# bababyVN/medical-image-segmentation-and-classification

Measured on AMD Instinct MI355X. Metric: images/sec (train step) Attention U-Net 256x256 bs=32/GPU, higher is better.
Workload: dtype bf16; 1 GPU; AttentionUNet 256x256 train step (fwd+BCE+bwd+clip+AdamW), bs=32/GPU, NHWC bf16 activations, fp32 master weights; global_batch=32, parallelism=dp1, hip_graph=False, wgrad_side_stream=True, plan_replay=C (mi355_plan_run)

## Files before the change

### medical-image-segmentation-and-classification_amd/csrc/bn.hip

```cpp
#include "rowred.hpp"

template <typename T> struct BnStatsOp {
  static constexpr int NQ = 2;
  static constexpr bool WRITES = false;
  typedef double Acc;
  static constexpr int EPC = 16 / (int)sizeof(T);
  const T* x;
  int ld;
  __device__ void load_cols(int) {}
  __device__ void apply(size_t row, int c0, Acc (&acc)[NQ][EPC]) const {
    const Vec16<T> v = ld16<T>(x + row * ld + c0);
#pragma unroll
    for (int e = 0; e < EPC; ++e) {
      const double f = (double)to_f32<T>(v.v[e]);
      acc[0][e] += f;
      acc[1][e] += f * f;
    }
  }
};


template <int CH, int BL, int NQ>
__device__ __forceinline__ void fold_partials(const float* __restrict__ partial, int nblocks, int rowlen, const int (&off)[NQ], int C,
                                              double* red , double (&out)[NQ]) {
  static_assert(CH * BL == 1024 && CH <= 64 && (CH & (CH - 1)) == 0, "1024-thread workgroup, power-of-two channel count");
  const int cl = threadIdx.x % CH, bl = threadIdx.x / CH;
  const int c = blockIdx.x * CH + cl;
  const int wave = threadIdx.x >> 6, lane = threadIdx.x & 63;
  double s[NQ];
#pragma unroll
  for (int q = 0; q < NQ; ++q) {
    double s0 = 0, s1 = 0, s2 = 0, s3 = 0;
    if (c < C) {
      const float* p = partial + off[q] + c;
      int b = bl;
      for (; b + 3 * BL < nblocks; b += 4 * BL) {
        s0 += (double)p[(size_t)b * rowlen];
        s1 += (double)p[(size_t)(b + BL) * rowlen];
        s2 += (double)p[(size_t)(b + 2 * BL) * rowlen];
        s3 += (double)p[(size_t)(b + 3 * BL) * rowlen];
      }
      for (; b < nblocks; b += BL) s0 += (double)p[(size_t)b * rowlen];
    }
    s[q] = (s0 + s1) + (s2 + s3);
  }
#pragma unroll
  for (int q = 0; q < NQ; ++q) {
#pragma unroll
    for (int m = CH; m < 64; m <<= 1) s[q] += __shfl_xor(s[q], m, 64);
    if (lane < CH) red[(q * 16 + wave) * CH + lane] = s[q];
  }
  __syncthreads();
#pragma unroll
  for (int q = 0; q < NQ; ++q) {
    double t = 0;
    if (threadIdx.x < CH) {
#pragma unroll
      for (int w = 0; w < 16; ++w) t += red[(q * 16 + w) * CH + threadIdx.x];
    }
    out[q] = t;
  }
}

extern "C" int mi355_rowreduce_blocks(long long M) { return rowreduce_blocks(M); }

extern "C" int mi355_bn_stats(const void* x, float* partial, long long M, int C, int ld, int dtype, mi355_stream_t s) {
  MI355_CHECK_ARG(x && partial && M > 0, "bn_stats: bad arguments");
  return dispatch_dtype(dtype, "bn_stats", [&](auto tag) {
    using T = decltype(tag);
    BnStatsOp<T> op{(const T*)x, ld};
    return rowred_launch<T>(op, M, C, partial, (hipStream_t)s);
  });
}

template <int CH, int BL>
__global__ __launch_bounds__(1024) void bn_finalize_kernel(const float* __restrict__ partial, int nblocks, double M, int C,
                                   const float* __restrict__ gamma, const float* __restrict__ beta,
                                   float* __restrict__ rmean, float* __restrict__ rvar, int64_t* nbt, float momentum,
                                   float eps, float* __restrict__ scale, float* __restrict__ shift,
                                   float* __restrict__ mean_out, float* __restrict__ invstd_out) {
  __shared__ double red[2 * 16 * CH];
  double sums2[2];
  fold_partials<CH, BL, 2>(partial, nblocks, 2 * C, {0, C}, C, red, sums2);
  const double s = sums2[0], q = sums2[1];
  const int c = blockIdx.x * CH + threadIdx.x;
  if (threadIdx.x >= CH) return;
  if (c == 0 && nbt) *nbt += 1;
  if (c >= C) return;
  const double mean = s / M;
  double var = q / M - mean * mean;
  if (var < 0) var = 0;
  const float invstd = (float)(1.0 / sqrt(var + (double)eps));
  if (rmean) {
    const double unb = M > 1 ? var * M / (M - 1) : var;
    rmean[c] = (float)((1.0 - momentum) * rmean[c] + momentum * mean);
    rvar[c] = (float)((1.0 - momentum) * rvar[c] + momentum * unb);
  }
  const float sc = gamma[c] * invstd;
  scale[c] = sc;
  shift[c] = beta[c] - (float)mean * sc;
  mean_out[c] = (float)mean;
  invstd_out[c] = invstd;
}

extern "C" int mi355_bn_finalize(const float* partial, int nblocks, long long M, int C, const float* gamma,
                                 const float* beta, float* running_mean, float* running_var, int64_t* nbt,
                                 float momentum, float eps, float* scale, float* shift, float* mean, float* invstd,
                                 mi355_stream_t s) {
  MI355_CHECK_ARG(partial && gamma && beta && scale && shift && mean && invstd, "bn_finalize: null pointer");
  if (nblocks > 128)
    hipLaunchKernelGGL((bn_finalize_kernel<4, 256>), dim3(ceil_div(C, 4)), dim3(1024), 0, (hipStream_t)s, partial, nblocks, (double)M, C,
                       gamma, beta, running_mean, running_var, nbt, momentum, eps, scale, shift, mean, invstd);
  else
    hipLaunchKernelGGL((bn_finalize_kernel<32, 32>), dim3(ceil_div(C, 32)), dim3(1024), 0, (hipStream_t)s, partial, nblocks, (double)M, C,
                       gamma, beta, running_mean, running_var, nbt, momentum, eps, scale, shift, mean, invstd);
  MI355_LAUNCH_CHECK();
  return MI355_OK;
}

__global__ __launch_bounds__(256) void fold_rows_kernel(const float* __restrict__ in, int rows, int rowlen, float* __restrict__ out,
                                                        int nsplit) {
  __shared__ double red[4][64];
  const int cl = threadIdx.x & 63, rl = threadIdx.x >> 6;
  const int c = blockIdx.x * 64 + cl;
  const int per = (rows + nsplit - 1) / nsplit;
  const int r0 = blockIdx.y * per, r1 = min(rows, r0 + per);
  double s0 = 0, s1 = 0, s2 = 0, s3 = 0;
  if (c < rowlen) {
    int r = r0 + rl;
    for (; r + 12 < r1; r += 16) {
      s0 += (double)in[(size_t)r * rowlen + c];
      s1 += (double)in[(size_t)(r + 4) * rowlen + c];
      s2 += (double)in[(size_t)(r + 8) * rowlen + c];
      s3 += (double)in[(size_t)(r + 12) * rowlen + c];
    }
    for (; r < r1; r += 4) s0 += (double)in[(size_t)r * rowlen + c];
  }
  red[rl][cl] = (s0 + s1) + (s2 + s3);
  __syncthreads();
  if (rl == 0 && c < rowlen) out[(size_t)blockIdx.y * rowlen + c] = (float)((red[0][cl] + red[1][cl]) + (red[2][cl] + red[3][cl]));
}

extern "C" int mi355_fold_rows(const float* partial, int rows, int rowlen, float* out, int nsplit, mi355_stream_t s) {
  MI355_CHECK_ARG(partial && out && rows > 0 && rowlen > 0 && nsplit > 0 && nsplit <= rows, "fold_rows: bad arguments");
  hipLaunchKernelGGL(fold_rows_kernel, dim3(ceil_div(rowlen, 64), nsplit), dim3(256), 0, (hipStream_t)s, partial, rows, rowlen, out,
                     nsplit);
  MI355_LAUNCH_CHECK();
  return MI355_OK;
}

__global__ void bn_eval_coeffs_kernel(const float* gamma, const float* beta, const float* rm, const float* rv, float eps,
                                      int C, float* scale, float* shift) {
  const int c = blockIdx.x * blockDim.x + threadIdx.x;
  if (c >= C) return;
  const float sc = gamma[c] / sqrtf(rv[c] + eps);
  scale[c] = sc;
  shift[c] = beta[c] - rm[c] * sc;
}

__global__ void bn_fold_bias_kernel(const float* bias, const float* scale, const float* shift, float* out, int C) {
  const int c = blockIdx.x * blockDim.x + threadIdx.x;
  if (c < C) out[c] = scale[c] * (bias ? bias[c] : 0.f) + shift[c];
}

extern "C" int mi355_bn_fold_bias(const float* bias, const float* scale, const float* shift, float* out, int C, mi355_stream_t s) {
  MI355_CHECK_ARG(scale && shift && out && C > 0, "bn_fold_bias: bad arguments");
  hipLaunchKernelGGL(bn_fold_bias_kernel, dim3(ceil_div(C, 128)), dim3(128), 0, (hipStream_t)s, bias, scale, shift, out, C);
  MI355_LAUNCH_CHECK();
  return MI355_OK;
}

extern "C" int mi355_bn_eval_coeffs(const float* gamma, const float* beta, const float* running_mean,
                                    const float* running_var, float eps, int C, float* scale, float* shift,
                                    mi355_stream_t s) {
  hipLaunchKernelGGL(bn_eval_coeffs_kernel, dim3(ceil_div(C, 128)), dim3(128), 0, (hipStream_t)s, gamma, beta, running_mean,
                     running_var, eps, C, scale, shift);
  MI355_LAUNCH_CHECK();
  return MI355_OK;
}

template <typename T, bool H2 = false, bool HR = false> struct BnActOp {
  static constexpr int EPC = 16 / (int)sizeof(T);
  const T* x; int ldx; const float* scale; const float* shift;
  const T* x2; int ldx2; const float* scale2; const float* shift2;
  const T* res; int ldr;
  T* y; int ldy;
  int act;
  float sc[EPC], sh[EPC], sc2[EPC];
  __device__ void load_cols(int c0) {
#pragma unroll
    for (int e = 0; e < EPC; ++e) {
      sc[e] = scale ? scale[c0 + e] : 1.f;
      sh[e] = scale ? shift[c0 + e] : 0.f;
      sc2[e] = H2 ? scale2[c0 + e] : 0.f;
      if constexpr (H2) sh[e] += shift2[c0 + e];
    }
  }
#ifndef BN_ACT_FETCH
#define BN_ACT_FETCH 8
#endif
  static constexpr int FETCH_ROWS = BN_ACT_FETCH;
  struct In { Vec16<T> v, v2, vr; };
  __device__ In fetch(size_t row, int c0) const {
    In in;
    in.v = ld16_nt<T>(x + row * ldx + c0);
    if constexpr (H2) in.v2 = ld16<T>(x2 + row * ldx2 + c0);
    if constexpr (HR) in.vr = ld16<T>(res + row * ldr + c0);
    return in;
  }
  __device__ void pin(In& in) const {
    pin16(in.v);
    if constexpr (H2) pin16(in.v2);
    if constexpr (HR) pin16(in.vr);
  }
  __device__ void finish(const In& in, size_t row, int c0) const {
    float f[EPC];
#pragma unroll
    for (int e = 0; e < EPC; ++e) f[e] = __builtin_fmaf(to_f32<T>(in.v.v[e]), sc[e], sh[e]);
    if constexpr (H2) {
#pragma unroll
      for (int e = 0; e < EPC; ++e) f[e] = __builtin_fmaf(to_f32<T>(in.v2.v[e]), sc2[e], f[e]);
    }
    const bool relu = act & 1, post = act & 2;
    Vec16<T> o;
#pragma unroll
    for (int e = 0; e < EPC; ++e) {
      float v = f[e];
      if (HR && !post) v += to_f32<T>(in.vr.v[e]);
      if (relu) v = fmaxf(v, 0.f);
      if (HR && post) v += to_f32<T>(in.vr.v[e]);
      o.v[e] = from_f32<T>(v);
    }
    st16<T>(y + row * ldy + c0, o);
  }
};

extern "C" int mi355_bn_act(const void* x, int ldx, const float* scale, const float* shift, const void* x2, int ldx2,
                            const float* scale2, const float* shift2, const void* res, int ldr, void* y, int ldy,
                            long long M, int C, int act, int dtype, mi355_stream_t s) {
  MI355_CHECK_ARG(x && y && M > 0, "bn_act: bad arguments");
  MI355_CHECK_ARG(!x2 || (scale2 && shift2), "bn_act: second operand needs scale2/shift2");
  return dispatch_dtype(dtype, "bn_act", [&](auto tag) {
    using T = decltype(tag);
    auto run = [&](auto op) {
      op.x = (const T*)x; op.ldx = ldx; op.scale = scale; op.shift = shift; op.x2 = (const T*)x2; op.ldx2 = ldx2;
      op.scale2 = scale2; op.shift2 = shift2; op.res = (const T*)res; op.ldr = ldr; op.y = (T*)y; op.ldy = ldy; op.act = act;
      return rowmap_launch<T>(op, M, C, (hipStream_t)s);
    };
    if (x2) return res ? run(BnActOp<T, true, true>{}) : run(BnActOp<T, true, false>{});
    return res ? run(BnActOp<T, false, true>{}) : run(BnActOp<T, false, false>{});
  });
}

#ifndef BN_ACT_POOL_WGS
#define BN_ACT_POOL_WGS 16
#endif
template <typename T, bool HR>
__global__ __launch_bounds__(256) void bn_act_pool2_kernel(const T* __restrict__ x, int ldx, const float* __restrict__ scale,
                                                           const float* __restrict__ shift, T* __restrict__ y, int ldy,
                                                           T* __restrict__ p, int ldp, int N, int H, int W, int C, int act,
                                                           const T* __restrict__ res = nullptr, int ldr = 0) {
  constexpr int EPC = 16 / (int)sizeof(T);
  const int cp = C / EPC, Ho = H >> 1, Wo = W >> 1;
  const long long total = (long long)N * Ho * Wo * cp;
  for (long long i = (long long)blockIdx.x * blockDim.x + threadIdx.x; i < total; i += (long long)gridDim.x * blockDim.x) {
    const int c0 = (int)(i % cp) * EPC;
    long long q = i / cp;
    const int wo = (int)(q % Wo); q /= Wo;
    const int ho = (int)(q % Ho);
    const int n = (int)(q / Ho);
    float sc[EPC], sh[EPC], m[EPC];
#pragma unroll
    for (int e = 0; e < EPC; ++e) { sc[e] = scale[c0 + e]; sh[e] = shift[c0 + e]; }
    const size_t r0 = ((size_t)(n * H + 2 * ho) * W + 2 * wo);
    Vec16<T> in[4];
#pragma unroll
    for (int k = 0; k < 4; ++k)
      in[k] = ld16_nt<T>(x + (r0 + (size_t)(k >> 1) * W + (k & 1)) * ldx + c0);
    Vec16<T> rs[4];
    if constexpr (HR) {
#pragma unroll
      for (int k = 0; k < 4; ++k) rs[k] = ld16<T>(res + (r0 + (size_t)(k >> 1) * W + (k & 1)) * ldr + c0);
    }
#pragma unroll
    for (int k = 0; k < 4; ++k) {
      Vec16<T> o;
#pragma unroll
      for (int e = 0; e < EPC; ++e) {
        float v = __builtin_fmaf(to_f32<T>(in[k].v[e]), sc[e], sh[e]);
        if (HR && !(act & 2)) v += to_f32<T>(rs[k].v[e]);
        if (act & 1) v = fmaxf(v, 0.f);
        if (HR && (act & 2)) v += to_f32<T>(rs[k].v[e]);
        o.v[e] = from_f32<T>(v);
        const float r = to_f32<T>(o.v[e]);
        m[e] = k == 0 ? r : fmaxf(m[e], r);
      }
      st16<T>(y + (r0 + (size_t)(k >> 1) * W + (k & 1)) * ldy + c0, o);
    }
    if (p) {
      Vec16<T> o;
#pragma unroll
      for (int e = 0; e < EPC; ++e) o.v[e] = from_f32<T>(m[e]);
      st16<T>(p + ((size_t)(n * Ho + ho) * Wo + wo) * ldp + c0, o);
    }
  }
}

extern "C" int mi355_bn_act_pool2(const void* x, int ldx, const float* scale, const float* shift, void* y, int ldy, void* p, int ldp,
                                  int N, int H, int W, int C, int act, int dtype, mi355_stream_t s) {
  MI355_CHECK_ARG(x && scale && shift && y && N > 0, "bn_act_pool2: bad arguments");
  MI355_CHECK_ARG(H % 2 == 0 && W % 2 == 0, "bn_act_pool2: %d x %d is not divisible into 2 x 2 groups", H, W);
  const int epc = dtype_is_2byte(dtype) ? 8 : 4;
  MI355_CHECK_ARG(C % epc == 0, "bn_act_pool2: C=%d must be a multiple of %d", C, epc);
  long long blocks = ((long long)N * (H / 2) * (W / 2) * (C / epc) + 255) / 256;
  if (blocks > 256 * BN_ACT_POOL_WGS) blocks = 256 * BN_ACT_POOL_WGS;
  return dispatch_dtype(dtype, "bn_act_pool2", [&](auto tag) {
    using T = decltype(tag);
    hipLaunchKernelGGL((bn_act_pool2_kernel<T, false>), dim3((int)blocks), dim3(256), 0, (hipStream_t)s, (const T*)x, ldx, scale, shift, (T*)y, ldy,
                       (T*)p, ldp, N, H, W, C, act);
    MI355_LAUNCH_CHECK();
    return (int)MI355_OK;
  });
}

extern "C" int mi355_bn_act_windows(const void* x, int ldx, const float* scale, const float* shift, const void* res, int ldr, void* y,
                                    int ldy, int N, int H, int W, int C, int act, int dtype, mi355_stream_t s) {
  MI355_CHECK_ARG(x && scale && shift && y && N > 0, "bn_act_windows: bad arguments");
  MI355_CHECK_ARG(H % 2 == 0 && W % 2 == 0, "bn_act_windows: %d x %d is not divisible into 2 x 2 groups", H, W);
  const int epc = dtype_is_2byte(dtype) ? 8 : 4;
  MI355_CHECK_ARG(C % epc == 0, "bn_act_windows: C=%d must be a multiple of %d", C, epc);
  long long blocks = ((long long)N * (H / 2) * (W / 2) * (C / epc) + 255) / 256;
  if (blocks > 256 * BN_ACT_POOL_WGS) blocks = 256 * BN_ACT_POOL_WGS;
  return dispatch_dtype(dtype, "bn_act_windows", [&](auto tag) {
    using T = decltype(tag);
    if (res)
      hipLaunchKernelGGL((bn_act_pool2_kernel<T, true>), dim3((int)blocks), dim3(256), 0, (hipStream_t)s, (const T*)x, ldx, scale, shift,
                         (T*)y, ldy, (T*)nullptr, 0, N, H, W, C, act, (const T*)res, ldr);
    else
      hipLaunchKernelGGL((bn_act_pool2_kernel<T, false>), dim3((int)blocks), dim3(256), 0, (hipStream_t)s, (const T*)x, ldx, scale, shift,
                         (T*)y, ldy, (T*)nullptr, 0, N, H, W, C, act, (const T*)nullptr, 0);
    MI355_LAUNCH_CHECK();
    return (int)MI355_OK;
  });
}

static inline long long bn_keep_limit() {
  static const long long mb = getenv("MI355_BN_KEEP_MB") ? atoll(getenv("MI355_BN_KEEP_MB")) : 0;
  return mb > 0 ? mb * 1000000ll : 0;
}
static inline int bn_reduce_keeps(long long bytes = 0) {
  static const int nt = getenv("MI355_BN_REDUCE_NT") ? atoi(getenv("MI355_BN_REDUCE_NT")) : 0;
  if (bn_keep_limit() && bytes > bn_keep_limit()) return 0;
  return nt ? 0 : 1;
}

static inline int bn_apply_keeps(long long bytes = 0) {
  static const int nt = getenv("MI355_BN_APPLY_NT") ? atoi(getenv("MI355_BN_APPLY_NT")) : 0;
  static const int lim = getenv("MI355_BN_KEEP_APPLY") ? atoi(getenv("MI355_BN_KEEP_APPLY")) : 0;
  if (lim && bn_keep_limit() && bytes > bn_keep_limit()) return 0;
  return nt ? 0 : 1;
}

static inline int bn_apply_reversed() {
  static const int rev = getenv("MI355_BN_APPLY_REV") ? atoi(getenv("MI355_BN_APPLY_REV")) : 0;
  return rev;
}

template <typename T, bool HASY = false, bool KEEP = true> struct BnBwdReduceOp {
  static constexpr int NQ = 2;
  static constexpr bool WRITES = false;
  typedef float Acc;
  static constexpr int EPC = 16 / (int)sizeof(T);
  const T* dy; int lddy; const T* y; int ldy; const T* x; int ldx;
  const float* mean; const float* invstd; const float* mscale; const float* mshift; int act;
  float mu[EPC], is[EPC], ms[EPC], mt[EPC];
  __device__ void load_cols(int c0) {
#pragma unroll
    for (int e = 0; e < EPC; ++e) {
      mu[e] = mean[c0 + e];
      is[e] = invstd[c0 + e];
      ms[e] = (act && !HASY) ? mscale[c0 + e] : 0.f;
      mt[e] = (act && !HASY) ? mshift[c0 + e] : 0.f;
    }
  }
#ifndef BN_RED_FETCH
#define BN_RED_FETCH 4
#endif
  static constexpr int FETCH_ROWS = BN_RED_FETCH;
#ifdef BN_RED_WGS
  static constexpr int MAX_WGS = BN_RED_WGS;
#endif
  struct In { Vec16<T> g, xv, yv; };
  __device__ In fetch(size_t row, int c0) const {
    In in;
    in.g = ld16_pol<KEEP, T>(dy + row * lddy + c0);
    in.xv = ld16_pol<KEEP, T>(x + row * ldx + c0);
    if constexpr (HASY) in.yv = ld16<T>(y + row * ldy + c0);
    return in;
  }
  __device__ void pin(In& in) const {
    pin16(in.g);
    pin16(in.xv);
    if constexpr (HASY) pin16(in.yv);
  }
  __device__ void finish(const In& in, size_t, int, Acc (&acc)[NQ][EPC]) const {
#pragma unroll
    for (int e = 0; e < EPC; ++e) {
      float gg = to_f32<T>(in.g.v[e]);
      const float xf = to_f32<T>(in.xv.v[e]);
      if (act) {
        const bool on = HASY ? (to_f32<T>(in.yv.v[e]) > 0.f) : (__builtin_fmaf(xf, ms[e], mt[e]) > 0.f);
        if (!on) gg = 0.f;
      }
      acc[0][e] += gg;
      acc[1][e] += gg * (xf - mu[e]) * is[e];
    }
  }
};

extern "C" int mi355_bn_bwd_reduce_rows(long long M) { return rowred_grid<BnBwdReduceOp<bf16_t>>(M); }

extern "C" int mi355_bn_bwd_reduce(const void* dy, int lddy, const void* y, int ldy, const void* x, int ldx,
                                   const float* mean, const float* invstd, const float* mscale, const float* mshift,
                                   float* partial, long long M, int C, int act, int dtype, mi355_stream_t s) {
  MI355_CHECK_ARG(dy && x && mean && invstd && partial && (!act || y || (mscale && mshift)), "bn_bwd_reduce: null pointer");
  return dispatch_dtype(dtype, "bn_bwd_reduce", [&](auto tag) {
    using T = decltype(tag);
    const bool keep = bn_reduce_keeps(2ll * M * C * (long long)sizeof(T)), hasy = act && y;
    auto run = [&](auto op) {
      op.dy = (const T*)dy; op.lddy = lddy; op.y = (const T*)y; op.ldy = ldy; op.x = (const T*)x; op.ldx = ldx;
      op.mean = mean; op.invstd = invstd; op.mscale = mscale; op.mshift = mshift; op.act = act;
      return rowred_launch<T>(op, M, C, partial, (hipStream_t)s);
    };
    if (hasy) return keep ? run(BnBwdReduceOp<T, true, true>{}) : run(BnBwdReduceOp<T, true, false>{});
    return keep ? run(BnBwdReduceOp<T, false, true>{}) : run(BnBwdReduceOp<T, false, false>{});
  });
}

template <int CH, int BL>
__global__ __launch_bounds__(1024) void bn_bwd_finalize_kernel(const float* __restrict__ partial, int nblocks, int C,
                                                               float* __restrict__ sums, float* __restrict__ dgamma,
                                                               float* __restrict__ dbeta, float accf, int nq, int q0, int q1) {
  __shared__ double red[2 * 16 * CH];
  double sums2[2];
  fold_partials<CH, BL, 2>(partial, nblocks, nq * C, {q0 * C, q1 * C}, C, red, sums2);
  const double s0 = sums2[0], s1 = sums2[1];
  const int c = blockIdx.x * CH + threadIdx.x;
  if (threadIdx.x >= CH || c >= C) return;
  sums[c] = (float)s0;
  sums[C + c] = (float)s1;
  if (dbeta) dbeta[c] = (accf != 0.f ? accf * dbeta[c] : 0.f) + (float)s0;
  if (dgamma) dgamma[c] = (accf != 0.f ? accf * dgamma[c] : 0.f) + (float)s1;
}

extern "C" int mi355_bn_bwd_finalize_at(const float* partial, int nblocks, int nq, int q0, int q1, int C, float* sums, float* dgamma,
                                        float* dbeta, float acc, mi355_stream_t s) {
  MI355_CHECK_ARG(partial && sums, "bn_bwd_finalize: null pointer");
  MI355_CHECK_ARG(nq >= 2 && q0 >= 0 && q0 < nq && q1 >= 0 && q1 < nq, "bn_bwd_finalize: quantities %d, %d of %d per partial row", q0, q1, nq);
  if (nblocks > 128)
    hipLaunchKernelGGL((bn_bwd_finalize_kernel<4, 256>), dim3(ceil_div(C, 4)), dim3(1024), 0, (hipStream_t)s, partial, nblocks, C,
                       sums, dgamma, dbeta, acc, nq, q0, q1);
  else
    hipLaunchKernelGGL((bn_bwd_finalize_kernel<32, 32>), dim3(ceil_div(C, 32)), dim3(1024), 0, (hipStream_t)s, partial, nblocks, C,
                       sums, dgamma, dbeta, acc, nq, q0, q1);
  MI355_LAUNCH_CHECK();
  return MI355_OK;
}

extern "C" int mi355_bn_bwd_finalize(const float* partial, int nblocks, int C, float* sums, float* dgamma, float* dbeta,
                                     float acc, mi355_stream_t s) {
  return mi355_bn_bwd_finalize_at(partial, nblocks, 2, 0, 1, C, sums, dgamma, dbeta, acc, s);
}

template <typename T, int NEX = 0, bool HASY = false, bool PACC = false, bool KEEP = true> struct BnBwdApplyOp {
  static constexpr int NQ = 1;
  static constexpr bool WRITES = true;
  typedef float Acc;
  static constexpr int EPC = 16 / (int)sizeof(T);
  static constexpr int NEXA = NEX > 0 ? NEX : 1;
  const T* dy; int lddy; const T* y; int ldy; const T* x; int ldx;
  const float* gamma; const float* mean; const float* invstd; const float* mscale; const float* mshift; const float* sums;
  T* dx; int lddx; T* dres; int lddres; T* dpost; int lddpost; int post_acc;
  float invM; int C; int act;
  long long last;
  const T* ex[NEXA]; int ldex, nex;
  float mu[EPC], is[EPC], k0[EPC], k1[EPC], gi[EPC], ms[EPC], mt[EPC];
  __device__ void load_cols(int c0) {
#pragma unroll
    for (int e = 0; e < EPC; ++e) {
      ms[e] = (act && !y) ? mscale[c0 + e] : 0.f;
      mt[e] = (act && !y) ? mshift[c0 + e] : 0.f;
      mu[e] = mean[c0 + e];
      is[e] = invstd[c0 + e];
      gi[e] = gamma[c0 + e] * is[e];
      k0[e] = sums[c0 + e] * invM;
      k1[e] = sums[C + c0 + e] * invM;
    }
  }
#ifndef BN_APPLY_FETCH
#define BN_APPLY_FETCH 4
#endif
  static constexpr int FETCH_ROWS = NEX > 0 ? 2 : BN_APPLY_FETCH;
  struct In { Vec16<T> g, xv, yv, pv, ev[NEXA]; };
  __device__ In fetch(size_t row, int c0) const {
    In in;
    if (last >= 0) row = (size_t)last - row;
    in.g = ld16_pol<KEEP, T>(dy + row * lddy + c0);
    in.xv = ld16_pol<KEEP, T>(x + row * ldx + c0);
    if constexpr (HASY) in.yv = ld16<T>(y + row * ldy + c0);
    if constexpr (PACC) in.pv = ld16<T>(dpost + row * lddpost + c0);
    if constexpr (NEX > 0) {
#pragma unroll
      for (int j = 0; j < NEX; ++j) in.ev[j] = ld16_nt<T>(ex[j] + row * ldex + c0);
    }
    return in;
  }
  __device__ void pin(In& in) const {
    pin16(in.g);
    pin16(in.xv);
    if constexpr (HASY) pin16(in.yv);
    if constexpr (PACC) pin16(in.pv);
    if constexpr (NEX > 0) {
#pragma unroll
      for (int j = 0; j < NEX; ++j) pin16(in.ev[j]);
    }
  }
  __device__ void finish(const In& in, size_t row, int c0, Acc (&acc)[NQ][EPC]) const {
    if (last >= 0) row = (size_t)last - row;
    if (dpost) {
      Vec16<T> pg = in.g;
      if constexpr (PACC || NEX > 0) {
#pragma unroll
        for (int e = 0; e < EPC; ++e) {
          float v = to_f32<T>(in.g.v[e]);
          if constexpr (PACC) v += to_f32<T>(in.pv.v[e]);
          if constexpr (NEX > 0) {
#pragma unroll
            for (int j = 0; j < NEX; ++j)
              if (j < nex) v += to_f32<T>(in.ev[j].v[e]);
          }
          pg.v[e] = from_f32<T>(v);
        }
      }
      st16<T>(dpost + row * lddpost + c0, pg);
    }
    Vec16<T> o, r;
#pragma unroll
    for (int e = 0; e < EPC; ++e) {
      float gg = to_f32<T>(in.g.v[e]);
      const float xf = to_f32<T>(in.xv.v[e]);
      if (act) {
        const bool on = HASY ? (to_f32<T>(in.yv.v[e]) > 0.f) : (__builtin_fmaf(xf, ms[e], mt[e]) > 0.f);
        if (!on) gg = 0.f;
      }
      const float xh = (xf - mu[e]) * is[e];
      const float d = bn_dx(gi[e], gg, k0[e], xh, k1[e]);
      o.v[e] = from_f32<T>(d);
      r.v[e] = from_f32<T>(gg);
      acc[0][e] += d;
    }
    st16<T>(dx + row * lddx + c0, o);
    if (dres) st16<T>(dres + row * lddres + c0, r);
  }
};

template <typename T, int NEX, bool HASY, bool PACC, bool KEEP>
static int bn_bwd_apply_launch(const void* dy, int lddy, const void* y, int ldy, const void* x, int ldx,
                               const float* gamma, const float* mean, const float* invstd, const float* mscale,
                               const float* mshift, const float* sums, void* dx, int lddx, void* dres, int lddres,
                               void* dpost, int lddpost, const void* const* ex, int ldex,
                               float* dbias_partial, long long M, int C, int act, mi355_stream_t s) {
  const float invM = (float)(1.0 / (double)M);
  const long long last = bn_apply_reversed() ? M - 1 : -1ll;
  BnBwdApplyOp<T, NEX, HASY, PACC, KEEP> op{(const T*)dy, lddy, (const T*)y, ldy, (const T*)x, ldx, gamma, mean, invstd,
                                            mscale, mshift, sums, (T*)dx, lddx, (T*)dres, lddres, (T*)dpost, lddpost, PACC ? 1 : 0, invM, C,
                                            act, last, {nullptr}, ldex, 0};
  if constexpr (NEX > 0) {
    for (int j = 0; j < NEX; ++j) {
      op.ex[j] = (const T*)(ex[j] ? ex[j] : ex[0]);
      if (ex[j]) op.nex = j + 1;
    }
  }
  return rowred_launch<T>(op, M, C, dbias_partial, (hipStream_t)s);
}

static int bn_bwd_apply_impl(const void* dy, int lddy, const void* y, int ldy, const void* x, int ldx,
                             const float* gamma, const float* mean, const float* invstd, const float* mscale,
                             const float* mshift, const float* sums, void* dx, int lddx, void* dres, int lddres,
                             void* dpost, int lddpost, int post_acc, const void* const* ex, int ldex,
                             float* dbias_partial, long long M, int C, int act, int dtype, mi355_stream_t s) {
  MI355_CHECK_ARG(dy && x && gamma && mean && invstd && sums && dx && (!act || y || (mscale && mshift)), "bn_bwd_apply: null pointer");
  if (ex) {
    for (int j = 1; j < 4; ++j) MI355_CHECK_ARG(!ex[j] || ex[j - 1], "bn_bwd_apply_post4: the earlier gradients must be given without gaps");
  }
  return dispatch_dtype(dtype, "bn_bwd_apply", [&](auto tag) {
    using T = decltype(tag);
    const bool hasy = act && y, pacc = dpost && post_acc;
    const bool keep = bn_apply_keeps(2ll * M * C * (long long)sizeof(T));
#define MI355_APPLY(NEX, HASY, PACC)                                                                                                       \
  (keep ? bn_bwd_apply_launch<T, NEX, HASY, PACC, true>(dy, lddy, y, ldy, x, ldx, gamma, mean, invstd, mscale, mshift, sums, dx, lddx,     \
                                                        dres, lddres, dpost, lddpost, ex, ldex, dbias_partial, M, C, act, s)               \
        : bn_bwd_apply_launch<T, NEX, HASY, PACC, false>(dy, lddy, y, ldy, x, ldx, gamma, mean, invstd, mscale, mshift, sums, dx, lddx,    \
                                                         dres, lddres, dpost, lddpost, ex, ldex, dbias_partial, M, C, act, s))
    if (ex) {
      if (hasy) return pacc ? MI355_APPLY(4, true, true) : MI355_APPLY(4, true, false);
      return pacc ? MI355_APPLY(4, false, true) : MI355_APPLY(4, false, false);
    }
    if (hasy) return pacc ? MI355_APPLY(0, true, true) : MI355_APPLY(0, true, false);
    return pacc ? MI355_APPLY(0, false, true) : MI355_APPLY(0, false, false);
#undef MI355_APPLY
  });
}

extern "C" int mi355_bn_bwd_apply(const void* dy, int lddy, const void* y, int ldy, const void* x, int ldx,
                                  const float* gamma, const float* mean, const float* invstd, const float* mscale,
                                  const float* mshift, const float* sums, void* dx, int lddx, void* dres, int lddres,
                                  void* dpost, int lddpost, int post_acc,
                                  float* dbias_partial, long long M, int C, int act, int dtype, mi355_stream_t s) {
  return bn_bwd_apply_impl(dy, lddy, y, ldy, x, ldx, gamma, mean, invstd, mscale, mshift, sums, dx, lddx, dres, lddres, dpost, lddpost,
                           post_acc, nullptr, 0, dbias_partial, M, C, act, dtype, s);
}

extern "C" int mi355_bn_bwd_apply_post4(const void* dy, int lddy, const void* y, int ldy, const void* x, int ldx,
                                        const float* gamma, const float* mean, const float* invstd, const float* mscale,
                                        const float* mshift, const float* sums, void* dx, int lddx, void* dpost, int lddpost,
                                        int post_acc, const void* ex0, const void* ex1, const void* ex2, const void* ex3, int ldex,
                                        long long M, int C, int act, int dtype, mi355_stream_t s) {
  MI355_CHECK_ARG(dpost && ex0, "bn_bwd_apply_post4: the post-activation operand's gradient and at least one earlier gradient expected");
  const void* ex[4] = {ex0, ex1, ex2, ex3};
  return bn_bwd_apply_impl(dy, lddy, y, ldy, x, ldx, gamma, mean, invstd, mscale, mshift, sums, dx, lddx, nullptr, 0, dpost, lddpost,
                           post_acc, ex, ldex, nullptr, M, C, act, dtype, s);
}

template <typename T, bool HASDY, bool KEEP> struct BnBwdPool2 {
  static constexpr int EPC = 16 / (int)sizeof(T);
  const T* dy; int lddy; const T* dp; int lddp; const T* x; int ldx;
  const float* mean; const float* invstd; const float* mscale; const float* mshift;
  int W, lrp, lwb;
  float mu[EPC], is[EPC], ms[EPC], mt[EPC];
  __device__ void load_common(int c0) {
#pragma unroll
    for (int e = 0; e < EPC; ++e) { mu[e] = mean[c0 + e]; is[e] = invstd[c0 + e]; ms[e] = mscale[c0 + e]; mt[e] = mshift[c0 + e]; }
  }
  struct Px { size_t pix[4]; Vec16<T> gv[4], xv[4], pv; };
  __device__ void fetch(long long r, int ty, int c0, Px& p) const {
    const long long q = r >> (lrp + 2);
    const long long R = q >> lwb;
    const int wcol = ((int)(q & ((1 << lwb) - 1)) << lrp) + ty;
#pragma unroll
    for (int b = 0; b < 4; ++b) p.pix[b] = (size_t)(2 * R + (b >> 1)) * W + 2 * wcol + (b & 1);
#pragma unroll
    for (int b = 0; b < 4; ++b) {
      if constexpr (HASDY) p.gv[b] = ld16_pol<KEEP, T>(dy + p.pix[b] * lddy + c0);
      p.xv[b] = ld16_pol<KEEP, T>(x + p.pix[b] * ldx + c0);
    }
    p.pv = ld16_pol<KEEP, T>(dp + ((size_t)R * (W >> 1) + wcol) * lddp + c0);
  }
  __device__ void pin(Px& p) const {
#pragma unroll
    for (int b = 0; b < 4; ++b) {
      if constexpr (HASDY) pin16(p.gv[b]);
      pin16(p.xv[b]);
    }
    pin16(p.pv);
  }
  __device__ void grads(const Px& p, int e, float (&g)[4]) const {
    float a[4];
#pragma unroll
    for (int b = 0; b < 4; ++b) a[b] = to_f32<T>(from_f32<T>(fmaxf(__builtin_fmaf(to_f32<T>(p.xv[b].v[e]), ms[e], mt[e]), 0.f)));
    const float mx = fmaxf(fmaxf(a[0], a[1]), fmaxf(a[2], a[3]));
    const bool w0 = a[0] == mx, w1 = !w0 && a[1] == mx, w2 = !(w0 || w1) && a[2] == mx, w3 = !(w0 || w1 || w2);
    const float pg = to_f32<T>(p.pv.v[e]);
    const bool win[4] = {w0, w1, w2, w3};
#pragma unroll
    for (int b = 0; b < 4; ++b) {
      const float t = (HASDY ? to_f32<T>(p.gv[b].v[e]) : 0.f) + (win[b] ? pg : 0.f);
      g[b] = a[b] > 0.f ? t : 0.f;
    }
  }
};

template <typename T, bool HASDY, bool KEEP = true> struct BnBwdReducePool2Op : BnBwdPool2<T, HASDY, KEEP> {
  static constexpr int NQ = 2;
  static constexpr bool WRITES = false;
  static constexpr int BATCH_ROWS = 4;
  typedef float Acc;
  static constexpr int EPC = 16 / (int)sizeof(T);
  __device__ void load_cols(int c0) { this->load_common(c0); }
  __device__ void finish(const typename BnBwdPool2<T, HASDY, KEEP>::Px& p, int, int, Acc (&acc)[NQ][EPC]) const {
#pragma unroll
    for (int e = 0; e < EPC; ++e) {
      float g[4];
      this->grads(p, e, g);
#pragma unroll
      for (int b = 0; b < 4; ++b) {
        acc[0][e] += g[b];
        acc[1][e] += g[b] * (to_f32<T>(p.xv[b].v[e]) - this->mu[e]) * this->is[e];
      }
    }
  }
};

template <typename T, bool HASDY, bool KEEP = true> struct BnBwdApplyPool2Op : BnBwdPool2<T, HASDY, KEEP> {
  static constexpr int NQ = 1;
  static constexpr bool WRITES = true;
  static constexpr int BATCH_ROWS = 4;
  typedef float Acc;
  static constexpr int EPC = 16 / (int)sizeof(T);
  const float* gamma; const float* sums; T* dx; int lddx; float invM; int C;
  float k0[EPC], k1[EPC], gi[EPC];
  __device__ void load_cols(int c0) {
    this->load_common(c0);
#pragma unroll
    for (int e = 0; e < EPC; ++e) {
      gi[e] = gamma[c0 + e] * this->is[e];
      k0[e] = sums[c0 + e] * invM;
      k1[e] = sums[C + c0 + e] * invM;
    }
  }
  __device__ void finish(const typename BnBwdPool2<T, HASDY, KEEP>::Px& p, int, int c0, Acc (&acc)[NQ][EPC]) const {
    Vec16<T> o[4];
#pragma unroll
    for (int e = 0; e < EPC; ++e) {
      float g[4];
      this->grads(p, e, g);
#pragma unroll
      for (int b = 0; b < 4; ++b) {
        const float xh = (to_f32<T>(p.xv[b].v[e]) - this->mu[e]) * this->is[e];
        const float d = bn_dx(gi[e], g[b], k0[e], xh, k1[e]);
        o[b].v[e] = from_f32<T>(d);
        acc[0][e] += d;
      }
    }
#pragma unroll
    for (int b = 0; b < 4; ++b) st16<T>(dx + p.pix[b] * lddx + c0, o[b]);
  }
};

static inline int exact_log2(long long v) {
  if (v <= 0 || (v & (v - 1))) return -1;
  int l = 0;
  while ((1LL << l) < v) ++l;
  return l;
}

extern "C" int mi355_bn_bwd_reduce_pool2_rows(long long M) { return rowred_grid<BnBwdReducePool2Op<bf16_t, true>>(M); }

extern "C" int mi355_bn_bwd_pool2_ok(int H, int W, int C, int dtype) {
  const int epc = dtype_is_2byte(dtype) ? 8 : 4;
  if (C % epc || H % 2 || W % 2) return 0;
  const int tpr = C / epc;
  if (tpr > 256 || exact_log2(tpr) < 0) return 0;
  const int rp = 256 / tpr;
  return W % (2 * rp) == 0 && exact_log2(W / (2 * rp)) >= 0;
}

template <typename T, typename Op> static void fill_pool2(Op& op, const void* dy, int lddy, const void* dp, int lddp, const void* x, int ldx,
                                                          const float* mean, const float* invstd, const float* mscale,
                                                          const float* mshift, int W, int C) {
  const int tpr = C / (16 / (int)sizeof(T)), rp = 256 / tpr;
  op.dy = (const T*)dy; op.lddy = lddy; op.dp = (const T*)dp; op.lddp = lddp; op.x = (const T*)x; op.ldx = ldx;
  op.mean = mean; op.invstd = invstd; op.mscale = mscale; op.mshift = mshift;
  op.W = W; op.lrp = exact_log2(rp); op.lwb = exact_log2(W / (2 * rp));
}

extern "C" int mi355_bn_bwd_reduce_pool2(const void* dy, int lddy, const void* dp, int lddp, const void* x, int ldx, const float* mean,
                                         const float* invstd, const float* mscale, const float* mshift, float* partial,
                                         int N, int H, int W, int C, int dtype, mi355_stream_t s) {
  MI355_CHECK_ARG(dp && x && mean && invstd && mscale && mshift && partial && N > 0, "bn_bwd_reduce_pool2: null pointer");
  MI355_CHECK_ARG(mi355_bn_bwd_pool2_ok(H, W, C, dtype), "bn_bwd_reduce_pool2: %d x %d x %d is not a geometry of the window-ordered pass", H, W, C);
  return dispatch_dtype(dtype, "bn_bwd_reduce_pool2", [&](auto tag) {
    using T = decltype(tag);
    auto run = [&](auto op) {
      fill_pool2<T>(op, dy, lddy, dp, lddp, x, ldx, mean, invstd, mscale, mshift, W, C);
      return rowred_launch<T>(op, (long long)N * H * W, C, partial, (hipStream_t)s);
    };
    const bool keep = bn_reduce_keeps(2ll * N * H * W * C * (long long)sizeof(T));
    if (dy) return keep ? run(BnBwdReducePool2Op<T, true, true>{}) : run(BnBwdReducePool2Op<T, true, false>{});
    return keep ? run(BnBwdReducePool2Op<T, false, true>{}) : run(BnBwdReducePool2Op<T, false, false>{});
  });
}

extern "C" int mi355_bn_bwd_apply_pool2(const void* dy, int lddy, const void* dp, int lddp, const void* x, int ldx, const float* gamma,
                                        const float* mean, const float* invstd, const float* mscale, const float* mshift,
                                        const float* sums, void* dx, int lddx, int N, int H, int W, int C, int dtype, mi355_stream_t s) {
  MI355_CHECK_ARG(dp && x && gamma && mean && invstd && mscale && mshift && sums && dx && N > 0, "bn_bwd_apply_pool2: null pointer");
  MI355_CHECK_ARG(mi355_bn_bwd_pool2_ok(H, W, C, dtype), "bn_bwd_apply_pool2: %d x %d x %d is not a geometry of the window-ordered pass", H, W, C);
  const long long M = (long long)N * H * W;
  return dispatch_dtype(dtype, "bn_bwd_apply_pool2", [&](auto tag) {
    using T = decltype(tag);
    auto run = [&](auto op) {
      fill_pool2<T>(op, dy, lddy, dp, lddp, x, ldx, mean, invstd, mscale, mshift, W, C);
      op.gamma = gamma; op.sums = sums; op.dx = (T*)dx; op.lddx = lddx; op.invM = (float)(1.0 / (double)M); op.C = C;
      return rowred_launch<T>(op, M, C, nullptr, (hipStream_t)s);
    };
    const bool keep = bn_apply_keeps(2ll * M * C * (long long)sizeof(T));
    if (dy) return keep ? run(BnBwdApplyPool2Op<T, true, true>{}) : run(BnBwdApplyPool2Op<T, true, false>{});
    return keep ? run(BnBwdApplyPool2Op<T, false, true>{}) : run(BnBwdApplyPool2Op<T, false, false>{});
  });
}

template <typename T> struct ColSumOp {
  static constexpr int NQ = 1;
  static constexpr bool WRITES = false;
  typedef float Acc;
  static constexpr int EPC = 16 / (int)sizeof(T);
  const T* x; int ld;
  __device__ void load_cols(int) {}
  __device__ void apply(size_t row, int c0, Acc (&acc)[NQ][EPC]) const {
    const Vec16<T> v = ld16<T>(x + row * ld + c0);
#pragma unroll
    for (int e = 0; e < EPC; ++e) acc[0][e] += to_f32<T>(v.v[e]);
  }
};

extern "C" int mi355_colsum(const void* x, int ld, float* partial, long long M, int C, int dtype, mi355_stream_t s) {
  MI355_CHECK_ARG(x && partial, "colsum: null pointer");
  return dispatch_dtype(dtype, "colsum", [&](auto tag) {
    using T = decltype(tag);
    ColSumOp<T> op{(const T*)x, ld};
    return rowred_launch<T>(op, M, C, partial, (hipStream_t)s);
  });
}

__global__ void colsum_finalize_kernel(const float* __restrict__ partial, int nblocks, int stride, int C,
                                       float* __restrict__ out, float accf) {
  __shared__ double red[16 * 32];
  double sums1[1];
  fold_partials<32, 32, 1>(partial, nblocks, stride * C, {0}, C, red, sums1);
  const double s0 = sums1[0];
  const int c = blockIdx.x * 32 + threadIdx.x;
  if (threadIdx.x >= 32 || c >= C) return;
  out[c] = (accf != 0.f ? accf * out[c] : 0.f) + (float)s0;
}

extern "C" int mi355_colsum_finalize(const float* partial, int nblocks, int stride, int C, float* out, float acc,
                                     mi355_stream_t s) {
  MI355_CHECK_ARG(partial && out, "colsum_finalize: null pointer");
  hipLaunchKernelGGL(colsum_finalize_kernel, dim3(ceil_div(C, 32)), dim3(1024), 0, (hipStream_t)s, partial, nblocks, stride, C,
                     out, acc);
  MI355_LAUNCH_CHECK();
  return MI355_OK;
}
```

### medical-image-segmentation-and-classification_amd/csrc/rowred.hpp

```cpp
#pragma once
#include <stdlib.h>
#include <type_traits>
#include "common.hpp"

#define MI355_RR_MAX_BLOCKS 1024

static inline int rowreduce_blocks(long long M) {
  long long b = (M + 63) / 64;
  if (b < 1) b = 1;
  if (b > MI355_RR_MAX_BLOCKS) b = MI355_RR_MAX_BLOCKS;
  return (int)b;
}

struct RowRedGeom {
  long long M;
  int C;
  int rows_per_block;
  int tpr;
  int rp;
  int nb_rows;
};

template <typename T>
static inline RowRedGeom rowred_geom(long long M, int C, int nblocks) {
  RowRedGeom g;
  const int epc = 16 / (int)sizeof(T);
  const int cp = C / epc;
  g.M = M;
  g.C = C;
  g.rows_per_block = (int)((M + nblocks - 1) / nblocks);
  g.tpr = cp < 256 ? cp : 256;
  g.rp = 256 / g.tpr;
  return g;
}

template <typename Op, typename = void> struct has_max_wgs : std::false_type {};
template <typename Op> struct has_max_wgs<Op, std::void_t<decltype(Op::MAX_WGS)>> : std::true_type {};
template <typename Op, typename = void> struct has_fetch : std::false_type {};
template <typename Op> struct has_fetch<Op, std::void_t<typename Op::In>> : std::true_type {};
template <typename Op, typename = void> struct has_batch : std::false_type {};
template <typename Op, typename X, typename = void> struct has_pin : std::false_type {};
template <typename Op, typename X> struct has_pin<Op, X, std::void_t<decltype(std::declval<const Op&>().pin(std::declval<X&>()))>> : std::true_type {};
template <typename V> __device__ __forceinline__ void pin16(V& v) {
  static_assert(sizeof(V) == 16, "a 16-byte load result");
  typedef unsigned u32x4_t __attribute__((ext_vector_type(4)));
  u32x4_t w = __builtin_bit_cast(u32x4_t, v);
  asm volatile("" : "+v"(w) : : "memory");
  v = __builtin_bit_cast(V, w);
}
template <typename Op> struct has_batch<Op, std::void_t<decltype(Op::BATCH_ROWS)>> : std::true_type {};

template <typename T, typename Op>
__global__ __launch_bounds__(256) void rowred_kernel(Op op, RowRedGeom g, float* __restrict__ partial) {
  constexpr int EPC = 16 / (int)sizeof(T);
  constexpr int NQ = Op::NQ;
  typedef typename Op::Acc Acc;
  __shared__ Acc red[256 * NQ * EPC / 2 + 1];
  const int tid = threadIdx.x;
  const int tx = tid % g.tpr, ty = tid / g.tpr;
  const int chunk = blockIdx.y * 256 + tx;
  const int c0 = chunk * EPC;
  const bool active = ty < g.rp && c0 < g.C;
  Acc acc[NQ][EPC];
#pragma unroll
  for (int q = 0; q < NQ; ++q)
#pragma unroll
    for (int e = 0; e < EPC; ++e) acc[q][e] = 0;
  if (active) {
    op.load_cols(c0);
    const long long r0 = (long long)blockIdx.x * g.rows_per_block;
    long long r1 = r0 + g.rows_per_block;
    if (r1 > g.M) r1 = g.M;
    if constexpr (has_batch<Op>::value) {
      constexpr int B = Op::BATCH_ROWS;
      const long long st = (long long)gridDim.x * g.rp * B;
      long long r = (long long)blockIdx.x * g.rp * B;
#ifndef RR_NO_RING
      if (r < g.M) {
        typename Op::Px p;
        op.fetch(r, ty, c0, p);
        for (;;) {
          const long long rn = r + st;
          const bool more = rn < g.M;
          if constexpr (has_pin<Op, typename Op::Px>::value) op.pin(p);
          typename Op::Px cur = p;
          op.fetch(more ? rn : r, ty, c0, p);
          op.finish(cur, ty, c0, acc);
          r = rn;
          if (!more) break;
        }
      }
#else
      for (; r < g.M; r += st) {
        typename Op::Px p;
        op.fetch(r, ty, c0, p);
        if constexpr (has_pin<Op, typename Op::Px>::value) op.pin(p);
        op.finish(p, ty, c0, acc);
      }
#endif
    } else if constexpr (has_fetch<Op>::value) {
      constexpr int B = Op::FETCH_ROWS;
      const long long st = (long long)gridDim.x * g.rp * B;
      long long r = (long long)blockIdx.x * g.rp * B + ty;
#ifndef RR_NO_RING
      if (r + (long long)(B - 1) * g.rp < g.M) {
        typename Op::In in[B];
#pragma unroll
        for (int b = 0; b < B; ++b) in[b] = op.fetch((size_t)(r + (long long)b * g.rp), c0);
        for (;;) {
          const long long rn = r + st;
          const bool more = rn + (long long)(B - 1) * g.rp < g.M;
          const long long rf = more ? rn : r;
#pragma unroll
          for (int b = 0; b < B; ++b) {
            if constexpr (has_pin<Op, typename Op::In>::value) op.pin(in[b]);
            const typename Op::In cur = in[b];
            in[b] = op.fetch((size_t)(rf + (long long)b * g.rp), c0);
            op.finish(cur, (size_t)(r + (long long)b * g.rp), c0, acc);
          }
          r = rn;
          if (!more) break;
        }
      }
      for (long long q = r; q < g.M; q += g.rp) op.finish(op.fetch((size_t)q, c0), (size_t)q, c0, acc);
#else
      for (; r < g.M; r += st) {
        if (r + (long long)(B - 1) * g.rp < g.M) {
          typename Op::In in[B];
#pragma unroll
          for (int b = 0; b < B; ++b) in[b] = op.fetch((size_t)(r + (long long)b * g.rp), c0);
#pragma unroll
          for (int b = 0; b < B; ++b) {
            if constexpr (has_pin<Op, typename Op::In>::value) op.pin(in[b]);
            op.finish(in[b], (size_t)(r + (long long)b * g.rp), c0, acc);
          }
        } else {
          for (long long q = r; q < g.M; q += g.rp) op.finish(op.fetch((size_t)q, c0), (size_t)q, c0, acc);
        }
      }
#endif
    } else if constexpr (!Op::WRITES && sizeof(typename Op::Acc) == 4) {
#pragma unroll 2
      for (long long r = r0 + ty; r < r1; r += g.rp) op.apply((size_t)r, c0, acc);
    } else {
      for (long long r = r0 + ty; r < r1; r += g.rp) op.apply((size_t)r, c0, acc);
    }
  }
  for (int stride = 1; stride < g.rp; stride <<= 1) {
    const bool sender = active && (ty % (2 * stride)) == stride;
    const bool recver = active && (ty % (2 * stride)) == 0 && (ty + stride) < g.rp;
    __syncthreads();
    if (sender) {
      Acc* dst = red + (size_t)(((ty - stride) / (2 * stride)) * g.tpr + tx) * NQ * EPC;
#pragma unroll
      for (int q = 0; q < NQ; ++q)
#pragma unroll
        for (int e = 0; e < EPC; ++e) dst[q * EPC + e] = acc[q][e];
    }
    __syncthreads();
    if (recver) {
      const Acc* src = red + (size_t)((ty / (2 * stride)) * g.tpr + tx) * NQ * EPC;
#pragma unroll
      for (int q = 0; q < NQ; ++q)
#pragma unroll
        for (int e = 0; e < EPC; ++e) acc[q][e] += src[q * EPC + e];
    }
  }
  if (active && ty == 0 && partial) {
#pragma unroll
    for (int q = 0; q < NQ; ++q)
#pragma unroll
      for (int e = 0; e < EPC; ++e) partial[((size_t)blockIdx.x * NQ + q) * g.C + c0 + e] = (float)acc[q][e];
    for (int b = blockIdx.x + gridDim.x; b < g.nb_rows; b += gridDim.x)
#pragma unroll
      for (int q = 0; q < NQ; ++q)
#pragma unroll
        for (int e = 0; e < EPC; ++e) partial[((size_t)b * NQ + q) * g.C + c0 + e] = 0.f;
  }
}

template <typename Op> static inline int rowred_grid(long long M) {
  int nb = rowreduce_blocks(M);
  static const int rr_wgs = getenv("MI355_RR_WGS") ? atoi(getenv("MI355_RR_WGS")) : 0;
  if constexpr (has_fetch<Op>::value || has_batch<Op>::value) {
    int cap = 256;
    if constexpr (has_max_wgs<Op>::value) cap = Op::MAX_WGS;
    if (rr_wgs > 0) cap = rr_wgs;
    nb = nb < cap ? nb : cap;
  }
  return nb;
}

template <typename T, typename Op>
static inline int rowred_launch(const Op& op, long long M, int C, float* partial, hipStream_t s) {
  const int epc = 16 / (int)sizeof(T);
  if (C % epc != 0) {
    mi355_set_error("row reduction: C=%d must be a multiple of %d", C, epc);
    return MI355_ERR_ARG;
  }
  const int nb_rows = rowreduce_blocks(M);
  const int nb = rowred_grid<Op>(M);
  RowRedGeom g = rowred_geom<T>(M, C, nb);
  g.nb_rows = nb_rows;
  const int cp = C / epc;
  dim3 grid(nb, (cp + 255) / 256);
  hipLaunchKernelGGL((rowred_kernel<T, Op>), grid, dim3(256), 0, s, op, g, partial);
  hipError_t e = hipGetLastError();
  if (e != hipSuccess) {
    mi355_set_error("row reduction launch failed: %s", hipGetErrorString(e));
    return (int)e;
  }
  return MI355_OK;
}

template <typename T, typename Op>
__global__ __launch_bounds__(256) void rowmap_kernel(Op op, long long M, int cp) {
  constexpr int EPC = 16 / (int)sizeof(T);
  const int tpr = cp < 256 ? cp : 256;
  const int rp = 256 / tpr;
  const int tx = threadIdx.x % tpr, ty = threadIdx.x / tpr;
  if (ty >= rp) return;
  for (int c = tx; c < cp; c += tpr) {
    op.load_cols(c * EPC);
    if constexpr (has_fetch<Op>::value) {
      constexpr int B = Op::FETCH_ROWS;
      const long long st = (long long)gridDim.x * rp * B;
      for (long long r = (long long)blockIdx.x * rp * B + ty; r < M; r += st) {
        if (r + (long long)(B - 1) * rp < M) {
          typename Op::In in[B];
#pragma unroll
          for (int b = 0; b < B; ++b) in[b] = op.fetch((size_t)(r + b * rp), c * EPC);
#pragma unroll
          for (int b = 0; b < B; ++b) {
            if constexpr (has_pin<Op, typename Op::In>::value) op.pin(in[b]);
            op.finish(in[b], (size_t)(r + b * rp), c * EPC);
          }
        } else {
          for (long long q = r; q < M; q += rp) op.finish(op.fetch((size_t)q, c * EPC), (size_t)q, c * EPC);
        }
      }
    } else {
      for (long long r = (long long)blockIdx.x * rp + ty; r < M; r += (long long)gridDim.x * rp) op.apply((size_t)r, c * EPC);
    }
  }
}

template <typename T, typename Op>
static inline int rowmap_launch(const Op& op, long long M, int C, hipStream_t s) {
  const int epc = 16 / (int)sizeof(T);
  if (C % epc != 0) {
    mi355_set_error("elementwise: C=%d must be a multiple of %d", C, epc);
    return MI355_ERR_ARG;
  }
  const int cp = C / epc;
  const int rp = 256 / (cp < 256 ? cp : 256);
  long long rpb = rp;
  if constexpr (has_fetch<Op>::value) rpb *= Op::FETCH_ROWS;
  long long blocks = (M + rpb - 1) / rpb;
  static const int rm_wgs = getenv("MI355_RM_WGS") ? atoi(getenv("MI355_RM_WGS")) : 256 * 4;
  const long long cap = has_fetch<Op>::value ? rm_wgs : 256 * 16;
  if (blocks > cap) blocks = cap;
  if (blocks < 1) blocks = 1;
  hipLaunchKernelGGL((rowmap_kernel<T, Op>), dim3((int)blocks), dim3(256), 0, s, op, M, cp);
  hipError_t e = hipGetLastError();
  if (e != hipSuccess) {
    mi355_set_error("elementwise launch failed: %s", hipGetErrorString(e));
    return (int)e;
  }
  return MI355_OK;
}
```

Before: 2147 images/s.

## Issue first row fetches before column loads and resize grid for small BN applies

BN backward reduce and apply ops now issue their first ring of row loads before loading the per-column statistics, clamping out-of-range rows to the last row, so global-load latency overlaps the column setup. The mscale/mshift loads become unconditional with a select, which removes a branch per element. For write-only (no partial) fetch ops on tensors under a size threshold, the grid is resized from occupancy so that row batches are spread evenly over a bounded number of slots. This adds a few redundant clamped loads and changes the grid size for small BN apply kernels.

```diff
diff --git a/medical-image-segmentation-and-classification_amd/csrc/bn.hip b/medical-image-segmentation-and-classification_amd/csrc/bn.hip
--- a/medical-image-segmentation-and-classification_amd/csrc/bn.hip
+++ b/medical-image-segmentation-and-classification_amd/csrc/bn.hip
@@ -375,18 +375,23 @@
   const float* mean; const float* invstd; const float* mscale; const float* mshift; int act;
   float mu[EPC], is[EPC], ms[EPC], mt[EPC];
   __device__ void load_cols(int c0) {
+    const bool remask = act && !HASY;
+    const float* msp = remask ? mscale : mean;
+    const float* mtp = remask ? mshift : mean;
 #pragma unroll
     for (int e = 0; e < EPC; ++e) {
       mu[e] = mean[c0 + e];
       is[e] = invstd[c0 + e];
-      ms[e] = (act && !HASY) ? mscale[c0 + e] : 0.f;
-      mt[e] = (act && !HASY) ? mshift[c0 + e] : 0.f;
+      const float a = msp[c0 + e], b = mtp[c0 + e];
+      ms[e] = remask ? a : 0.f;
+      mt[e] = remask ? b : 0.f;
     }
   }
 #ifndef BN_RED_FETCH
 #define BN_RED_FETCH 4
 #endif
   static constexpr int FETCH_ROWS = BN_RED_FETCH;
+  static constexpr bool FETCH_FIRST = true;
 #ifdef BN_RED_WGS
   static constexpr int MAX_WGS = BN_RED_WGS;
 #endif
@@ -486,10 +491,14 @@
   const T* ex[NEXA]; int ldex, nex;
   float mu[EPC], is[EPC], k0[EPC], k1[EPC], gi[EPC], ms[EPC], mt[EPC];
   __device__ void load_cols(int c0) {
-#pragma unroll
-    for (int e = 0; e < EPC; ++e) {
-      ms[e] = (act && !y) ? mscale[c0 + e] : 0.f;
-      mt[e] = (act && !y) ? mshift[c0 + e] : 0.f;
+    const bool remask = act && !y;
+    const float* msp = remask ? mscale : mean;
+    const float* mtp = remask ? mshift : mean;
+#pragma unroll
+    for (int e = 0; e < EPC; ++e) {
+      const float a = msp[c0 + e], b = mtp[c0 + e];
+      ms[e] = remask ? a : 0.f;
+      mt[e] = remask ? b : 0.f;
       mu[e] = mean[c0 + e];
       is[e] = invstd[c0 + e];
       gi[e] = gamma[c0 + e] * is[e];
@@ -501,6 +510,7 @@
 #define BN_APPLY_FETCH 4
 #endif
   static constexpr int FETCH_ROWS = NEX > 0 ? 2 : BN_APPLY_FETCH;
+  static constexpr bool FETCH_FIRST = true;
   struct In { Vec16<T> g, xv, yv, pv, ev[NEXA]; };
   __device__ In fetch(size_t row, int c0) const {
     In in;
diff --git a/medical-image-segmentation-and-classification_amd/csrc/rowred.hpp b/medical-image-segmentation-and-classification_amd/csrc/rowred.hpp
--- a/medical-image-segmentation-and-classification_amd/csrc/rowred.hpp
+++ b/medical-image-segmentation-and-classification_amd/csrc/rowred.hpp
@@ -49,6 +49,8 @@
   v = __builtin_bit_cast(V, w);
 }
 template <typename Op> struct has_batch<Op, std::void_t<decltype(Op::BATCH_ROWS)>> : std::true_type {};
+template <typename Op, typename = void> struct fetch_first : std::false_type {};
+template <typename Op> struct fetch_first<Op, std::void_t<decltype(Op::FETCH_FIRST)>> : std::bool_constant<Op::FETCH_FIRST> {};
 
 template <typename T, typename Op>
 __global__ __launch_bounds__(256) void rowred_kernel(Op op, RowRedGeom g, float* __restrict__ partial) {
@@ -66,8 +68,14 @@
   for (int q = 0; q < NQ; ++q)
 #pragma unroll
     for (int e = 0; e < EPC; ++e) acc[q][e] = 0;
-  if (active) {
-    op.load_cols(c0);
+#ifndef RR_NO_RING
+  constexpr bool FF = fetch_first<Op>::value;
+  static_assert(!FF || (has_fetch<Op>::value && !has_batch<Op>::value), "FETCH_FIRST: an op with fetch / finish");
+#else
+  constexpr bool FF = false;
+#endif
+  if (FF ? active && g.M > 0 : active) {
+    if constexpr (!FF) op.load_cols(c0);
     const long long r0 = (long long)blockIdx.x * g.rows_per_block;
     long long r1 = r0 + g.rows_per_block;
     if (r1 > g.M) r1 = g.M;
@@ -103,10 +111,21 @@
       const long long st = (long long)gridDim.x * g.rp * B;
       long long r = (long long)blockIdx.x * g.rp * B + ty;
 #ifndef RR_NO_RING
+      typename Op::In in[B];
+      if constexpr (FF) {
+        const long long rl = g.M - 1;
+#pragma unroll
+        for (int b = 0; b < B; ++b) {
+          const long long q = r + (long long)b * g.rp;
+          in[b] = op.fetch((size_t)(q < rl ? q : rl), c0);
+        }
+        op.load_cols(c0);
+      }
       if (r + (long long)(B - 1) * g.rp < g.M) {
-        typename Op::In in[B];
-#pragma unroll
-        for (int b = 0; b < B; ++b) in[b] = op.fetch((size_t)(r + (long long)b * g.rp), c0);
+        if constexpr (!FF) {
+#pragma unroll
+          for (int b = 0; b < B; ++b) in[b] = op.fetch((size_t)(r + (long long)b * g.rp), c0);
+        }
         for (;;) {
           const long long rn = r + st;
           const bool more = rn + (long long)(B - 1) * g.rp < g.M;
@@ -191,6 +210,32 @@
   return nb;
 }
 
+static inline long long rowred_small_limit() {
+  static const long long mb = getenv("MI355_RR_SMALL_MB") ? atoll(getenv("MI355_RR_SMALL_MB")) : 128;
+  return mb * (1ll << 20);
+}
+
+template <typename T, typename Op>
+static inline int rowred_stream_grid(long long M, int C, int nb_persistent) {
+  static const int rr_wgs = getenv("MI355_RR_WGS") ? atoi(getenv("MI355_RR_WGS")) : 0;
+  static const int per_cu_env = getenv("MI355_RR_SMALL_WGS") ? atoi(getenv("MI355_RR_SMALL_WGS")) : 0;
+  if (rr_wgs > 0 || M * (long long)C * (long long)sizeof(T) >= rowred_small_limit()) return nb_persistent;
+  static const int occ = [] {
+    int n = 0;
+    if (hipOccupancyMaxActiveBlocksPerMultiprocessor(&n, rowred_kernel<T, Op>, 256, 0) != hipSuccess || n < 1) n = 1;
+    return n;
+  }();
+  const int per_cu = per_cu_env > 0 ? per_cu_env : (occ < 2 ? occ : 2);
+  const int epc = 16 / (int)sizeof(T);
+  const int cp = C / epc, tpr = cp < 256 ? cp : 256, rp = 256 / tpr;
+  const int rows_b = rp * Op::FETCH_ROWS;
+  const long long batches = (M + rows_b - 1) / rows_b;
+  const long long slots = 256ll * per_cu / ((cp + 255) / 256);
+  const long long per_wg = (batches + slots - 1) / slots;
+  const long long nb = (batches + per_wg - 1) / per_wg;
+  return nb < 1 ? 1 : (int)nb;
+}
+
 template <typename T, typename Op>
 static inline int rowred_launch(const Op& op, long long M, int C, float* partial, hipStream_t s) {
   const int epc = 16 / (int)sizeof(T);
@@ -199,7 +244,10 @@
     return MI355_ERR_ARG;
   }
   const int nb_rows = rowreduce_blocks(M);
-  const int nb = rowred_grid<Op>(M);
+  int nb = rowred_grid<Op>(M);
+  if constexpr (has_fetch<Op>::value && !has_batch<Op>::value) {
+    if (!partial && M > 0) nb = rowred_stream_grid<T, Op>(M, C, nb);
+  }
   RowRedGeom g = rowred_geom<T>(M, C, nb);
   g.nb_rows = nb_rows;
   const int cp = C / epc;
```

Result: no change. 2144 images/s (-0.1%).
